# franciscotln/cosmology-model-fit

Hardware: AMD Instinct MI355X
Metric: walker-logL evals/s, Pantheon+ 1701-SN full-cov chi2, theta resident in HBM (higher is better)
Workload: dtype f64; 1 GPU; Pantheon+-shaped 1701-SN full-cov flat-LCDM chi2 + prior, 4096 walkers per GPU per step (BASELINE configs[1] at N=1), G=4000, theta resident in HBM; workload_key=pantheon, walkers_per_gpu=4096, walkers_total=4096, n_sn=1701, n_grid=4000, ndim=4, parallelism=walkers sharded over 1 GPU(s)

## Files before the change

cosmology-model-fit_amd/csrc/cosmofit_api.hip:

```cpp
#include <hip/hip_runtime.h>
#include <sys/prctl.h>

#include <cmath>
#include <cstdio>
#include <cstdlib>
#include <chrono>
#include <cstring>
#include <algorithm>
#include <atomic>
#include <utility>
#include <condition_variable>
#include <memory>
#include <mutex>
#include <string>
#include <thread>
#include <vector>

#include "../../include/cosmofit.h"
#include "cf_pack.h"
#include "cosmofit_device.h"

typedef double d2 __attribute__((ext_vector_type(2)));

#define CF_YPK_SLACK 8192
#define CF_DELTA_SLACK 4096

static long long cf_tune(const char* key, long long dflt) {
  static const std::string env = [] { const char* e = getenv("CF_TUNE"); return std::string(e ? e : ""); }();
  const size_t kl = strlen(key);
  for (size_t pos = 0; pos < env.size();) {
    const size_t end = std::min(env.find(',', pos), env.size());
    if (end - pos > kl + 1 && env.compare(pos, kl, key) == 0 && env[pos + kl] == '=') return atoll(env.c_str() + pos + kl + 1);
    pos = end + 1;
  }
  return dflt;
}

#define CF_BAO_NODES 6
#define CF_SN_PARTS_MAX 4
#define CF_SN_REC_SLACK (512 * CF_SN_PARTS_MAX)
template <int MODEL, int FDE>
__global__ void walker_kernel(cf_dev_desc d, const double* theta, int64_t W, double* delta, double* dm_out, double* mucorr_out,
                              d2* bao_nodes, d2* table_out);
template <int MODEL, int FDE>
__global__ void walker_fast_kernel(cf_walker_args d, const double* theta, int64_t W, double* delta, d2* bao_nodes, double* theta_copy,
                                   int frag_b, int sn_parts);
template <int MODEL, int FDE, int LANES, int ROLES>
__global__ void small_blocks_kernel(cf_dev_desc d, const double* theta, int64_t W, const d2* bao_nodes, double* chi2_extra,
                                    double* blocks_out, double* bao_out);
template <int MODEL, int FDE, int C>
__global__ void growth_kernel(cf_dev_desc d, const double* theta, int64_t W, const d2* aux_nodes, double* chi2_extra, int accumulate,
                              double* blocks_out, double* theory_out);
template <int MODEL, int FDE>
__global__ void hz_kernel(cf_dev_desc d, const double* theta, const double* z, int64_t n, double* out);
#define CF_DECLARE_GROWTH(M, F, C) \
  extern template __global__ void growth_kernel<M, F, C>(cf_dev_desc, const double*, int64_t, const d2*, double*, int, double*, double*);
#define CF_DECLARE_WALKER(M, F)                                                                                            \
  extern template __global__ void walker_kernel<M, F>(cf_dev_desc, const double*, int64_t, double*, double*, double*, d2*, d2*); \
  extern template __global__ void walker_fast_kernel<M, F>(cf_walker_args, const double*, int64_t, double*, d2*, double*, int, int); \
  extern template __global__ void small_blocks_kernel<M, F, 16, 1>(cf_dev_desc, const double*, int64_t, const d2*, double*, \
                                                                   double*, double*);                                      \
  extern template __global__ void small_blocks_kernel<M, F, 64, 1>(cf_dev_desc, const double*, int64_t, const d2*, double*, \
                                                                   double*, double*);                                      \
  extern template __global__ void small_blocks_kernel<M, F, 64, 2>(cf_dev_desc, const double*, int64_t, const d2*, double*, \
                                                                   double*, double*);                                      \
  extern template __global__ void hz_kernel<M, F>(cf_dev_desc, const double*, const double*, int64_t, double*);             \
  CF_DECLARE_GROWTH(M, F, 1) CF_DECLARE_GROWTH(M, F, 2) CF_DECLARE_GROWTH(M, F, 4) CF_DECLARE_GROWTH(M, F, 8)
CF_DECLARE_WALKER(0, 0) CF_DECLARE_WALKER(0, 1) CF_DECLARE_WALKER(0, 2) CF_DECLARE_WALKER(0, 3)
CF_DECLARE_WALKER(1, 0) CF_DECLARE_WALKER(1, 1) CF_DECLARE_WALKER(1, 2) CF_DECLARE_WALKER(1, 3)

typedef void (*walker_fn)(cf_dev_desc, const double*, int64_t, double*, double*, double*, d2*, d2*);
static walker_fn pick_walker(int model, int fde) {
  static const walker_fn table[2][4] = {
      {walker_kernel<0, 0>, walker_kernel<0, 1>, walker_kernel<0, 2>, walker_kernel<0, 3>},
      {walker_kernel<1, 0>, walker_kernel<1, 1>, walker_kernel<1, 2>, walker_kernel<1, 3>}};
  return table[model][fde];
}
typedef void (*walker_fast_fn)(cf_walker_args, const double*, int64_t, double*, d2*, double*, int, int);
static walker_fast_fn pick_walker_fast(int model, int fde) {
  static const walker_fast_fn table[2][4] = {
      {walker_fast_kernel<0, 0>, walker_fast_kernel<0, 1>, walker_fast_kernel<0, 2>, walker_fast_kernel<0, 3>},
      {walker_fast_kernel<1, 0>, walker_fast_kernel<1, 1>, walker_fast_kernel<1, 2>, walker_fast_kernel<1, 3>}};
  return table[model][fde];
}
static bool walker_fast_ok(const cf_dev_desc& d) {
  static const bool off = cf_tune("walker_generic", 0) != 0;
  return !off && d.chunk_shift == 3 && d.ndim <= 64 && !d.sn_fixed_mu && !d.sn_dir && !d.sn_vel_mult && (!d.sn_lin || d.lin_in_rec);
}
static cf_epilogue epilogue_of(const cf_dev_desc& d) {
  cf_epilogue e{};
  e.ndim = d.ndim; e.has_bounds = d.has_bounds; e.n_gauss = d.n_gauss; e.n_chi2_gauss = d.n_chi2_gauss;
  e.cpl_wall = d.cpl_wall; e.n_fs8 = d.n_fs8; e.n_cc = d.n_cc; e.cc_f_inverse = d.cc_f_inverse;
  e.log_norm = d.log_norm; e.logl_const = d.logl_const; e.cc_logdet = d.cc_logdet;
  e.w0 = d.slot[CF_P_W0_D]; e.wa = d.slot[CF_P_WA_D]; e.fs8err = d.slot[CF_P_FS8ERR_D]; e.fcc = d.slot[CF_P_FCC_D];
  for (int k = 0; k < CF_MAX_NDIM; ++k) { e.lo[k] = d.lo[k]; e.hi[k] = d.hi[k]; }
  for (int k = 0; k < CF_MAX_GAUSS; ++k) {
    e.gauss_idx[k] = d.gauss_idx[k]; e.gauss_mean[k] = d.gauss_mean[k]; e.gauss_sigma[k] = d.gauss_sigma[k];
    e.chi2_gauss_idx[k] = d.chi2_gauss_idx[k]; e.chi2_gauss_mean[k] = d.chi2_gauss_mean[k]; e.chi2_gauss_sigma[k] = d.chi2_gauss_sigma[k];
  }
  return e;
}
static cf_walker_args walker_args_of(const cf_dev_desc& d) {
  cf_walker_args a{};
  a.ndim = d.ndim; a.n_grid = d.n_grid; a.ez_model = d.ez_model; a.fde = d.fde;
  a.chunk_shift = d.chunk_shift; a.om_mode = d.om_mode;
  a.n_sn = d.n_sn; a.n_ld = d.n_ld;
  a.has_vstep = d.has_vstep; a.step_pm1 = d.step_pm1; a.lin_in_rec = d.lin_in_rec; a.n_aux = d.n_aux;
  a.z_max = d.z_max; a.step = d.step; a.c = d.c; a.inv_step = d.inv_step; a.inv_last = d.inv_last;
  a.or_h2 = d.or_h2; a.omnu_h2 = d.omnu_h2;
  for (int k = 0; k < CF_N_SLOTS; ++k) a.slot[k] = d.slot[k];
  a.sn_rec = d.sn_rec; a.log10_tab = d.log10_tab; a.nu_sw = d.nu_sw; a.ln_sw = d.ln_sw; a.exp2_tab = d.exp2_tab;
// ... 629 lines not shown
      if (c->solve_mode != CF_SOLVE_BLOCKED_TRSM) {
        cf_pack_inverse(c->sn_chol, c->n_sn, c->sn_chol_ld, prep.ip);
        const double inv_probe = cf_invpack_probe(prep.ip, c->sn_chol, c->sn_chol_ld);
        if (inv_probe <= limit) {
          prep.solve_mode = CF_SOLVE_INVERSE_GEMM;
          prep.probe_rel = inv_probe;
        } else if (c->solve_mode == CF_SOLVE_INVERSE_GEMM) {
          return bail(fail(CF_ERR_ILL_CONDITIONED, "cf_create: the explicit inverse of the factor disagrees with row-by-row forward "
                                                       "substitution by " + fmt_g(inv_probe) + " relative (limit " +
                                                       fmt_g(limit) + "); use CF_SOLVE_BLOCKED_TRSM or CF_SOLVE_AUTO for "
                                                       "this covariance"));
        } else {
          prep.solve_mode = CF_SOLVE_BLOCKED_TRSM;
          prep.ip = cf_host_invpack();
        }
      }
      if (prep.solve_mode == CF_SOLVE_BLOCKED_TRSM) {
        if (pack_default(c->sn_chol, c->n_sn, c->sn_chol_ld, prep.hp, &prep.probe_rel) != 0)
          return bail(fail(CF_ERR_NOT_POSDEF, "cf_create: the Cholesky factor has a non-positive or non-finite pivot"));
        if (!(prep.probe_rel <= CF_PROBE_LIMIT))
          return bail(fail(CF_ERR_ILL_CONDITIONED, "cf_create: the blocked solve disagrees with row-by-row forward substitution by " +
                                                       fmt_g(prep.probe_rel) + " relative on a probe vector (limit 1e-11): "
                                                       "the factor's diagonal blocks are too ill-conditioned for 256-row block inverses"));
      }
      prep.packed = true;
    }
    h->solve_mode = prep.solve_mode;
    h->pack_probe_rel = prep.probe_rel;
    if (h->solve_mode == CF_SOLVE_INVERSE_GEMM) {
      if ((rc = h->ipack.upload(prep.ip))) return bail(rc);
    } else {
      if ((rc = h->pack.upload(prep.hp))) return bail(rc);
    }
  }
  if (c->n_bao > 0) {
    int rc;
    if ((rc = upload_vec(h->bao_z, c->bao_z, c->n_bao))) return bail(rc);
    if ((rc = upload_vec(h->bao_val, c->bao_val, c->n_bao))) return bail(rc);
    if ((rc = upload_vec(h->bao_inv_cov, c->bao_inv_cov, (int64_t)c->n_bao * c->n_bao))) return bail(rc);
    if (h->bao_qty.ensure((size_t)c->n_bao * 4)) return bail(CF_ERR_HIP);
    if (hipMemcpy(h->bao_qty.p, c->bao_qty, (size_t)c->n_bao * 4, hipMemcpyHostToDevice) != hipSuccess)
      return bail(fail(CF_ERR_HIP, "hipMemcpy(bao_qty) failed"));
    d.bao_z = h->bao_z.as<const double>();
    d.bao_val = h->bao_val.as<const double>();
    d.bao_inv_cov = h->bao_inv_cov.as<const double>();
    d.bao_qty = h->bao_qty.as<const int32_t>();
  }
  if (d.n_aux > 0) {
    std::vector<int32_t> base((size_t)d.n_aux);
    for (int k = 0; k < d.n_aux; ++k) base[k] = aux_node_base(d, k < c->n_bao ? c->bao_z[k] : c->fs8_z[k - c->n_bao]);
    if (h->bao_base.ensure(base.size() * 4)) return bail(CF_ERR_HIP);
    if (hipMemcpy(h->bao_base.p, base.data(), base.size() * 4, hipMemcpyHostToDevice) != hipSuccess)
      return bail(fail(CF_ERR_HIP, "hipMemcpy(bao_base) failed"));
    d.bao_base = h->bao_base.as<const int32_t>();
  }
  if (c->n_fs8 > 0) {
    int rc;
    const int n = c->n_fs8;
    if ((rc = upload_vec(h->fs8_z, c->fs8_z, n))) return bail(rc);
    if ((rc = upload_vec(h->fs8_val, c->fs8_val, n))) return bail(rc);
    if ((rc = upload_vec(h->fs8_inv_cov, c->fs8_inv_cov, (int64_t)n * n))) return bail(rc);
    if ((rc = upload_vec(h->fs8_fid, c->fs8_fid, n))) return bail(rc);
    d.fs8_z = h->fs8_z.as<const double>();
    d.fs8_val = h->fs8_val.as<const double>();
    d.fs8_inv_cov = h->fs8_inv_cov.as<const double>();
    d.fs8_fid = h->fs8_fid.as<const double>();
// ... 389 lines not shown
    return a.frag_b ? launch_tri_gemm_small_t<16, true, 1>(a, st) : launch_tri_gemm_small_t<16, false, 1>(a, st);
  }
  if (a.frag_b) return fail(CF_ERR_INVALID, "internal: fragment-ordered residuals handed to the throughput solve kernel");
  return tri_gemm_panel_width(a.W) == 32 ? launch_tri_gemm_t<2, 2>(a, st) : launch_tri_gemm_t<1, 2>(a, st);
}

static int launch_eval(cf_handle* h, const double* th, int64_t Wc, double* out, int out_kind, hipStream_t st,
                       double* dm_out, double* mucorr_out, double* blocks_out, double* bao_out, double* chi2_sn_out,
                       hipEvent_t* ev, double* fs8_block_out = nullptr, double* fs8_theory_out = nullptr) {
  const cf_dev_desc& d = h->d;
  unsigned long long* nf = h->nonfinite.as<unsigned long long>();
  double* delta = h->delta.as<double>();
  d2* bao_nodes = h->bao_nodes.as<d2>();
  if (ev) HIP_TRY(hipEventRecord(ev[0], st));
  if (ev && !(h->d.n_sn > 0 || h->has_small_blocks || h->has_growth || h->qsr)) HIP_TRY(hipEventRecord(ev[1], st));
  const bool walker_work = d.n_sn > 0 || h->has_small_blocks || h->has_growth;
  double* extra = (h->has_small_blocks || h->has_growth || h->qsr) ? h->chi2_extra.as<double>() : nullptr;
  static const bool frag_env = cf_tune("small_frag", 1) != 0;
  const bool small_solve = d.n_sn > 0 && h->solve_mode == CF_SOLVE_INVERSE_GEMM && h->partial4.p && Wc <= small_batch_max();
  const bool frag_b = frag_env && small_solve && !dm_out && !mucorr_out && walker_fast_ok(d) && !h->qsr;
  if (h->qsr) {
    double* th_copy = h->theta_on_host ? h->theta.as<double>() : nullptr;
    int rc = cf_qsr_launch(h->qsr, th, Wc, delta, extra, out_kind, th_copy, st);
    if (rc) return rc;
    if (th_copy) th = th_copy;
    if (ev) HIP_TRY(hipEventRecord(ev[1], st));
  } else if (walker_work) {
    const size_t lds = ((size_t)d.n_grid + (d.n_grid >> d.chunk_shift) + 2) * 16;
    if (!dm_out && !mucorr_out && walker_fast_ok(d)) {
      double* th_copy = h->theta_on_host ? h->theta.as<double>() : nullptr;
      static const int parts_env = (int)cf_tune("sn_parts", 0);
      int sn_parts = parts_env > 0 ? parts_env : (Wc <= 64 ? 4 : (Wc <= 160 ? 2 : 1));
      if (sn_parts > CF_SN_PARTS_MAX || d.n_sn == 0) sn_parts = 1;
      hipLaunchKernelGGL(pick_walker_fast(d.ez_model, d.fde), dim3((unsigned)(Wc * sn_parts)), dim3(512), lds, st, walker_args_of(d), th,
                         Wc, delta, bao_nodes, th_copy, frag_b ? 1 : 0, sn_parts);
      if (th_copy) th = th_copy;
    } else
      hipLaunchKernelGGL(pick_walker(d.ez_model, d.fde), dim3((unsigned)Wc), dim3(512), lds, st, d, th, Wc, delta, dm_out, mucorr_out,
                         bao_nodes, (d2*)nullptr);
    if (ev) HIP_TRY(hipEventRecord(ev[1], st));
    if (h->has_small_blocks) {
      static const int64_t wide_max = cf_tune("sb_wide_max", 2048);
      static const int64_t roles_max = cf_tune("sb_roles_max", 2048);
      const int lanes = Wc <= wide_max ? 64 : 16, roles = (lanes == 64 && Wc <= roles_max) ? 2 : 1, per_wg = 256 / (lanes * roles);
      hipLaunchKernelGGL(pick_small_blocks(d.ez_model, d.fde, lanes, roles), dim3((unsigned)((Wc + per_wg - 1) / per_wg)), dim3(256), 0, st, d, th, Wc,
                         (const d2*)bao_nodes, extra, blocks_out, bao_out);
    }
    if (h->has_growth)
      hipLaunchKernelGGL(pick_growth(d.ez_model, d.fde, d.fs8_steps), dim3((unsigned)Wc), dim3(256),
                         (size_t)(2 * (d.fs8_steps + 1) + 16 + CF_MAX_FS8 + 2 + 256) * 8, st, d, th, Wc, (const d2*)bao_nodes, extra,
                         h->has_small_blocks ? 1 : 0, fs8_block_out, fs8_theory_out);
  }
  if (ev) HIP_TRY(hipEventRecord(ev[2], st));
  if (d.n_sn > 0 && h->solve_mode == CF_SOLVE_INVERSE_GEMM) {
    static const bool trim = cf_tune("gemm_trim", 1) != 0;
    const int n_rb_ = h->ipack.dev.n_rowblocks, nt_last = trim ? std::max(1, std::min(4, (d.n_pad - 64 * (n_rb_ - 1)) / 16)) : 4;
    static const int diag_skip = cf_tune("gemm_diag_skip", 1) != 0;
    TriGemmArgs a{h->epi.as<const cf_epilogue>(), h->ipack.dev.frags, d.n_ld, d.ndim, n_rb_, nt_last, diag_skip, th, Wc, delta,
                  h->max_walkers, h->partial.as<double>(), h->arrivals.as<unsigned int>(), extra, out,
                  out_kind, nf, chi2_sn_out, h->partial4.as<double>(), nullptr, 0ull, frag_b};
    if (h->theta_on_host && h->done_flags.p) {
      a.done_flag = (unsigned long long*)h->done_flags.p;
      a.done_seq = h->done_seq;
      const bool small = Wc <= small_batch_max() && a.partial4;
      const int pw = small ? 16 : tri_gemm_panel_width(Wc);
      h->done_armed = (int)((Wc + pw - 1) / pw);
      if (h->done_armed > CF_DONE_FLAGS) { a.done_flag = nullptr; h->done_armed = 0; }
    }
// ... 820 lines not shown
```

cosmology-model-fit_amd/csrc/cosmofit_device.h:

```cpp
#ifndef COSMOFIT_DEVICE_H
#define COSMOFIT_DEVICE_H

#include <stdint.h>

#define CF_MAX_NDIM 16
#define CF_MAX_GAUSS 8
#define CF_MAX_BAO 64
#define CF_MAX_GL 256
#define CF_MAX_CC 64
#define CF_MAX_FS8 64
#define CF_N_SLOTS 15

#define CF_BLOCK_TILES 16
#define CF_BLOCK_ROWS 256

#define CF_FDE_LCDM_D 0
#define CF_FDE_WCDM_D 1
#define CF_FDE_THAWING_D 2
#define CF_FDE_CPL_D 3

#define CF_EZ_LATE_FLAT_D 0
#define CF_EZ_PHYSICAL_D 1

#define CF_P_OFFSET_D 0
// ... 63 lines not shown
  const double* fs8_pts;
  const double* fs8_tab;
  int32_t n_aux, fs8_n_agrid;
  double or_h2, omnu_h2, o_gamma_h2, nu_m0, nu_rho0;
  double nu_qs_sq[5], nu_ws[5];
  const double* nu_grid;
  const double* ln_grid;
  const double* nu_sw;
  const double* ln_sw;
  const double* exp2_tab;
  int32_t n_bao, bao_dh_exact, rd_from_fit, rd_wm_late;
  const double* bao_z;
  const double* bao_val;
  const double* bao_inv_cov;
  const int32_t* bao_qty;
  const int32_t* bao_base;
  double rd_fit[11];
  int32_t cmb_mode, n_gl;
  const double* gl_x;
  const double* gl_w;
  double cmb_prior[3], cmb_inv_cov[9], zstar_fit[11];
  int32_t has_bounds, n_gauss, n_chi2_gauss, cpl_wall;
  double log_norm;
  int32_t sn_vel_mult, cc_f_inverse;
  double logl_const;
  double lo[CF_MAX_NDIM], hi[CF_MAX_NDIM];
  int32_t gauss_idx[CF_MAX_GAUSS];
  double gauss_mean[CF_MAX_GAUSS], gauss_sigma[CF_MAX_GAUSS];
  int32_t chi2_gauss_idx[CF_MAX_GAUSS];
  double chi2_gauss_mean[CF_MAX_GAUSS], chi2_gauss_sigma[CF_MAX_GAUSS];
};

struct cf_walker_args {
  int32_t ndim, n_grid, ez_model, fde;
  int32_t chunk_shift, om_mode;
  int32_t n_sn, n_ld;
  int32_t has_vstep, step_pm1, lin_in_rec, n_aux;
  double z_max, step, c, inv_step, inv_last;
  double or_h2, omnu_h2;
  cf_dev_slot slot[CF_N_SLOTS];
  const cf_d4* sn_rec;
  const void* log10_tab;
  const double* nu_sw;
  const double* ln_sw;
  const double* exp2_tab;
  const int32_t* bao_base;
};

struct cf_epilogue {
  int32_t ndim, has_bounds, n_gauss, n_chi2_gauss;
  int32_t cpl_wall, n_fs8, n_cc, cc_f_inverse;
  double log_norm, logl_const, cc_logdet;
  cf_dev_slot w0, wa, fs8err, fcc;
  double lo[CF_MAX_NDIM], hi[CF_MAX_NDIM];
  int32_t gauss_idx[CF_MAX_GAUSS];
  double gauss_mean[CF_MAX_GAUSS], gauss_sigma[CF_MAX_GAUSS];
  int32_t chi2_gauss_idx[CF_MAX_GAUSS];
  double chi2_gauss_mean[CF_MAX_GAUSS], chi2_gauss_sigma[CF_MAX_GAUSS];
};
#define CF_EPI_WORDS ((int)((sizeof(cf_epilogue) + 7) / 8))

struct cf_qsr_args {
  int32_t ndim, n_grid;
  int32_t n_sn, n_ld;
  int32_t n_qsr, two_grids;
  int32_t n_bao, n_bz;
  double c, fde_a;
  cf_dev_slot om, w0, h0, off_sn, off_q, scat, rd;
  const double* node_w;
  const double* node_zp3;
  const double* node_lnf;
  const int32_t* sn_j;
  const double* sn_t;
  const double* sn_h;
  const double* sn_zp1;
  const double* sn_obs;
  const int32_t* q_j;
  const double* q_t;
  const double* q_h;
// ... 63 lines not shown
```

cosmology-model-fit_amd/csrc/cosmofit_kernels.hip:

```cpp
#include <hip/hip_runtime.h>
#include <type_traits>
#include <stdint.h>

#include "cosmofit_device.h"
#include "cf_wave_scan.h"

typedef double d4 __attribute__((ext_vector_type(4)));
typedef double d2 __attribute__((ext_vector_type(2)));

#define CF_WAVE 64

__device__ __forceinline__ double slot_get(const cf_dev_desc& d, int s, const double* __restrict__ th) {
  const cf_dev_slot& p = d.slot[s];
  return p.idx >= 0 ? p.scale * th[p.idx] : p.fixed;
}

struct ThetaRow {
  double v;
};
__device__ __forceinline__ double readlane_f64(double v, int lane) {
  return __hiloint2double(__builtin_amdgcn_readlane(__double2hiint(v), lane), __builtin_amdgcn_readlane(__double2loint(v), lane));
}
template <class D>
__device__ __forceinline__ double slot_get(const D& d, int s, const ThetaRow& th) {
// ... 330 lines not shown
    double dx_max = 0.0;
#pragma unroll
    for (int k = 1; k < CH; ++k) {
      const double dx = x[k] - x[k - 1];
      dx_max = fmax(dx_max, fabs(dx));
      double p = fma(dx, 1.0 / 5040, 1.0 / 720);
      p = fma(p, dx, 1.0 / 120);
      p = fma(p, dx, 1.0 / 24);
      p = fma(p, dx, 1.0 / 6);
      p = fma(p, dx, 0.5);
      p = fma(p * dx, dx, dx);
      fde[k] = fma(fde[k - 1], p, fde[k - 1]);
    }
    if (!(dx_max < 0x1p-5)) {
#pragma unroll
      for (int k = 1; k < CH; ++k) fde[k] = exp_tab(x[k], etab);
    }
  }
#pragma unroll
  for (int k = 0; k < CH; ++k) {
    const int g = g0 + k;
    double z = (double)g * d.step;
    if (LAST) z = g >= G - 1 ? d.z_max : z;
    const double e2 = POWER_LAW ? e2_from_fde<MODEL>(wc, z, fde[k], nu_pre[k]) : e2_of_z<MODEL, FDE, true, D>(d, wc, z, nu_pre[k], ln[k], etab);
    const double v = c_over_H0 * rsqrt_pos(e2);
    dh[k] = (LAST && g >= G) ? 0.0 : v;
  }
  double prev = dpp_move<0x138, 0xF>(dh[CH - 1]);
  double run = 0.0;
  const double half = 0.5 * d.step;
#pragma unroll
  for (int k = 0; k < CH; ++k) {
    const bool counts = (k > 0 || lane > 0) && (!LAST || g0 + k < G);
    run = counts ? fma_vsv(prev + dh[k], half, run) : run;
    loc[k] = run;
    prev = dh[k];
  }
  return run;
}

template <int MODEL, int FDE, int CH, class D>
__device__ __forceinline__ void build_distance_table_regs(const D& d, const WalkerCosmo& wc, d2* tab,
                                                          d4* wave_pub, const double (&nu_pre)[CH], const double (&ln_pre)[CH],
                                                          const double* __restrict__ etab) {
  const int G = d.n_grid;
  const int tid = threadIdx.x, lane = tid & 63, wave = tid >> 6;
  const int g0 = tid * CH;
  const int base = g0 + tid;
  const double c_over_H0 = wc.c / wc.H0;
  double dh[CH], loc[CH];
  const int wave_last = (tid - lane) * CH + 64 * CH - 1;
  const double run = wave_last < G - 1 ? chunk_eval<MODEL, FDE, CH, false>(d, wc, c_over_H0, g0, lane, nu_pre, ln_pre, etab, dh, loc)
                                       : chunk_eval<MODEL, FDE, CH, true>(d, wc, c_over_H0, g0, lane, nu_pre, ln_pre, etab, dh, loc);
  const double incl = wave_inclusive_scan(run);
  const double first_dh = __hiloint2double(__builtin_amdgcn_readfirstlane(__double2hiint(dh[0])),
                                           __builtin_amdgcn_readfirstlane(__double2loint(dh[0])));
  if (lane == 63) wave_pub[wave] = (d4){incl, first_dh, dh[CH - 1], 0.0};
  __syncthreads();
  double term = 0.0;
  if (lane < CF_TPB_A / 64) {
    const d4 pv = wave_pub[lane];
    term = lane < wave ? pv[0] : 0.0;
    if (lane >= 1) {
      const int gb = lane * 64 * CH;
      const double zb = gb == G - 1 ? d.z_max : (double)gb * d.step;
      const double bnd = (wave_pub[lane - 1][2] + pv[1]) / 2 * (zb - (double)(gb - 1) * d.step);
      term += (lane <= wave && gb < G) ? bnd : 0.0;
// ... 87 lines not shown
template <class TAB>
__device__ double pchip_dh_tab(const TAB& T, double xi) {
  const int G = T.G;
  if (xi <= 0.0) return T.at(0).y;
  if (xi >= T.z_max) return T.at(G - 1).y;
  int i = (int)(xi * T.inv_step);
  i = i > G - 2 ? G - 2 : i;
  if (i > 0 && grid_z(i, G, T.step, T.z_max) >= xi) --i;
  if (i < G - 2 && grid_z(i + 1, G, T.step, T.z_max) < xi) ++i;
  const double x0 = grid_z(i, G, T.step, T.z_max);
  const double h_i = grid_z(i + 1, G, T.step, T.z_max) - x0;
  const double t = (xi - x0) / h_i;
  const double t2 = t * t, t3 = t2 * t;
  const double h00 = 2 * t3 - 3 * t2 + 1, h10 = t3 - 2 * t2 + t, h01 = -2 * t3 + 3 * t2, h11 = t3 - t2;
  return h00 * T.at(i).y + h10 * h_i * pchip_slope_tab(T, i) + h01 * T.at(i + 1).y + h11 * h_i * pchip_slope_tab(T, i + 1);
}

__device__ double z_star_fit(const double* f, double wb, double wm) {
  wb = pow(wb, f[2]);
  wm = pow(wm, f[3]);
  return pow(wm, f[4]) + f[0] * f[5] * pow(wb, f[6]) * pow(wm, f[7]) + f[1] * f[8] * pow(wm, f[9]) * pow(wb, f[10]);
}
__device__ double r_drag_fit(const double* f, double wb, double wm) {
  wb = pow(wb, f[0]);
  wm = pow(wm, f[1]);
  const double den = (f[2] * pow(wb, f[3])) + (f[4] * pow(wb, f[5]) * pow(wm, f[6])) + (f[7] * pow(wm, f[8]));
  return 1.0 / den - f[9] / pow(wm, f[10]);
}

template <bool FRAG>
__device__ __forceinline__ int delta_index(int i) {
  return FRAG ? ((i >> 3) * 128 + ((i >> 1) & 3) * 32 + (i & 1)) : i;
}
template <bool PM1, bool LIN = false, bool FRAG = false, class D = cf_dev_desc>
__device__ __forceinline__ void sn_fast_loop(const D& d, const DistTable& T, const d2* __restrict__ log_tab,
                                             double* __restrict__ out, double off, double v100, int tid, double lin = 0.0,
                                             int part = 0, int n_parts = 1) {
  const int n_sn = d.n_sn, first = part * CF_TPB_A + tid, stride = n_parts * CF_TPB_A;
  double r_pos = 1.0, r_neg = 1.0, c0 = 0.0;
  if (PM1 && d.has_vstep) {
    r_pos = 1.0 / (1.0 + v100 / d.c);
    r_neg = 1.0 / (1.0 + (-v100) / d.c);
    c0 = -1.0;
  }
  const d4* __restrict__ rec = reinterpret_cast<const d4*>(d.sn_rec) + first;
  if (part == 0 && tid < d.n_ld - n_sn) out[delta_index<FRAG>(n_sn + tid)] = 0.0;
  auto one_sn = [&](const d4& r, int i) {
    const double za = r[0], st = r[1], zhp1 = r[2], ob = r[3];
    double z_cosmo = za;
    if (!LIN && PM1) {
      z_cosmo = fma(za, st > 0.0 ? r_pos : r_neg, c0);
    } else if (!LIN && d.has_vstep) {
      const double z_pec = (v100 * st) / d.c;
      z_cosmo = -1.0 + za / (1.0 + z_pec);
    }
    const double off_i = LIN ? off + lin * st : off;
    out[delta_index<FRAG>(i)] = ob - off_i - fma_vsv(log10_tab(zhp1 * hermite_fast(T, z_cosmo), log_tab), 5.0, 25.0);
  };
  d4 ra = rec[0], rb;
  int i = first;
  while (i < n_sn) {
    rb = rec[stride];
    one_sn(ra, i);
    i += stride;
    if (i >= n_sn) break;
    rec += 2 * stride;
    ra = rec[0];
    one_sn(rb, i);
    i += stride;
  }
}

template <int MODEL, int FDE>
__global__ void __launch_bounds__(CF_TPB_A, 4)
walker_kernel(cf_dev_desc d, const double* __restrict__ theta, int64_t W, double* __restrict__ delta,
              double* __restrict__ dm_out, double* __restrict__ mucorr_out, d2* __restrict__ bao_nodes, d2* __restrict__ table_out) {
  extern __shared__ __align__(16) d2 lds_tab[];
  __shared__ __align__(16) d4 wave_pub[CF_TPB_A / 64];
  __shared__ __align__(16) d2 log_tab[64];
  __shared__ double exp2_tab[64];

  const int64_t w = blockIdx.x;
  if (w >= W) return;
  const double* th = theta + w * d.ndim;
  const int tid = threadIdx.x;
  if (tid < 64 && d.n_sn > 0) log_tab[tid] = reinterpret_cast<const d2*>(d.log10_tab)[tid];
  double nu_pre[8], ln_pre[8];
  constexpr bool POWER_LAW = FDE == CF_FDE_WCDM_D || FDE == CF_FDE_CPL_D;
#pragma unroll
  for (int k = 0; k < 8; ++k) {
    nu_pre[k] = (MODEL == CF_EZ_PHYSICAL_D && d.chunk_shift == 3) ? d.nu_sw[k * CF_TPB_A + tid] : -1.0;
    ln_pre[k] = (POWER_LAW && d.chunk_shift == 3) ? d.ln_sw[k * CF_TPB_A + tid] : -1.0;
  }
  if (POWER_LAW && d.chunk_shift == 3 && tid >= 64 && tid < 128) exp2_tab[tid - 64] = d.exp2_tab[tid - 64];
  if (POWER_LAW && d.chunk_shift == 3) __syncthreads();
  const WalkerCosmo wc = make_cosmo(d, th);
  DistTable T;
  T.tab = lds_tab;
  T.G = d.n_grid;
  T.chs = d.chunk_shift;
  T.step = d.step;
  T.inv_step = d.inv_step;
// ... 27 lines not shown
          double z_cosmo = zc;
          if (d.has_vstep) {
            const double v_km_s = d.sn_dir ? 100 * (d.sn_dir[3 * i] * vx + d.sn_dir[3 * i + 1] * vy + d.sn_dir[3 * i + 2] * vz) * d.sn_step[i]
                                           : v100 * d.sn_step[i];
            const double z_pec = v_km_s / d.c;
            z_cosmo = -1.0 + (1.0 + zc) / (1.0 + z_pec);
            if (d.sn_vel_mult) z_cosmo = fmax((1.0 + zc) * (1.0 + z_pec) - 1.0, 1e-8);
          }
          const double DMc = hermite_tab(T, z_cosmo);
          const double fixed = d.sn_fixed_mu ? d.sn_fixed_mu[i] : __longlong_as_double(0x7ff8000000000000ll);
          if (fixed == fixed) {
            const double DM = hermite_tab(T, zc);
            const double mu_corr = d.has_vstep ? 5.0 * log10_pos(DMc / DM) : 0.0;
            res = d.obs[i] - off_i - mu_corr - fixed;
            if (dm_out) dm_out[w * d.n_sn + i] = DM;
            if (mucorr_out) mucorr_out[w * d.n_sn + i] = mu_corr;
          } else if (!parts) {
            res = d.obs[i] - off_i - (25.0 + 5 * log10_pos((1.0 + d.z_hel[i]) * DMc));
          } else {
            const double DM = hermite_tab(T, zc);
            const double mu_corr = d.has_vstep ? 5.0 * log10(DMc / DM) : 0.0;
            const double mu_th = 25.0 + 5 * log10((1.0 + d.z_hel[i]) * DM);
            res = d.obs[i] - off_i - mu_corr - mu_th;
            if (dm_out) dm_out[w * d.n_sn + i] = DM;
            if (mucorr_out) mucorr_out[w * d.n_sn + i] = mu_corr;
          }
        }
        out[i] = res;
      }
    }
  }
}

template <int MODEL, int FDE>
__global__ void __launch_bounds__(CF_TPB_A, 4)
walker_fast_kernel(cf_walker_args d, const double* __restrict__ theta, int64_t W, double* __restrict__ delta,
                   d2* __restrict__ bao_nodes, double* __restrict__ theta_copy, int frag_b, int sn_parts) {
  extern __shared__ __align__(16) d2 lds_tab[];
  __shared__ __align__(16) d4 wave_pub[CF_TPB_A / 64];
  __shared__ __align__(16) d2 log_tab[64];
  __shared__ double exp2_all[CF_TPB_A / 64][64];

  const int64_t w = sn_parts > 1 ? blockIdx.x / (unsigned)sn_parts : blockIdx.x;
  const int part = sn_parts > 1 ? (int)(blockIdx.x % (unsigned)sn_parts) : 0;
  if (w >= W) return;
  const int tid = threadIdx.x, lane = tid & 63;
  double* const exp2_tab = exp2_all[tid >> 6];
  const ThetaRow th{theta[w * d.ndim + (lane < d.ndim ? lane : 0)]};
  if (theta_copy && part == 0 && tid < d.ndim) theta_copy[w * d.ndim + tid] = th.v;
  constexpr bool POWER_LAW = FDE == CF_FDE_WCDM_D || FDE == CF_FDE_CPL_D;
  d2 lt = (d2){0.0, 0.0};
  double et = 0.0;
  if (tid < 64 && d.n_sn > 0) lt = reinterpret_cast<const d2*>(d.log10_tab)[tid];
  if (POWER_LAW) et = d.exp2_tab[lane];
  double nu_pre[8], ln_pre[8];
#pragma unroll
  for (int k = 0; k < 8; ++k) {
    nu_pre[k] = MODEL == CF_EZ_PHYSICAL_D ? d.nu_sw[k * CF_TPB_A + tid] : -1.0;
    ln_pre[k] = POWER_LAW ? d.ln_sw[k * CF_TPB_A + tid] : -1.0;
  }
  if (tid < 64 && d.n_sn > 0) log_tab[tid] = lt;
  if (POWER_LAW) exp2_tab[lane] = et;
  const WalkerCosmo wc = make_cosmo(d, th);
  const double off = slot_get(d, CF_P_OFFSET_D, th);
  const double v100 = 100 * slot_get(d, CF_P_V_D, th);
  const double lin = d.lin_in_rec ? slot_get(d, CF_P_LIN_D, th) : 0.0;
  DistTable T;
  T.tab = lds_tab;
  T.G = d.n_grid;
  T.chs = 3;
  T.step = d.step;
  T.inv_step = d.inv_step;
  T.inv_last = d.inv_last;
  T.z_max = d.z_max;
  build_distance_table_regs<MODEL, FDE, 8>(d, wc, lds_tab, wave_pub, nu_pre, ln_pre, exp2_tab);
  for (int e = CF_TPB_A - 1 - tid; part == 0 && e < CF_BAO_NODES * d.n_aux; e += CF_TPB_A) {
    const int k = e / CF_BAO_NODES, o = e % CF_BAO_NODES;
    bao_nodes[(w * d.n_aux + k) * CF_BAO_NODES + o] = T.at(d.bao_base[k] + o);
  }
  if (d.n_sn > 0 && !frag_b) {
    double* out = delta + w * d.n_ld;
    if (d.lin_in_rec) sn_fast_loop<false, true>(d, T, log_tab, out, off, v100, tid, lin, part, sn_parts);
    else if (d.step_pm1) sn_fast_loop<true>(d, T, log_tab, out, off, v100, tid, 0.0, part, sn_parts);
    else sn_fast_loop<false>(d, T, log_tab, out, off, v100, tid, 0.0, part, sn_parts);
  } else if (d.n_sn > 0) {
    double* out = delta + (w >> 4) * (16 * (int64_t)d.n_ld) + 2 * (w & 15);
    if (d.lin_in_rec) sn_fast_loop<false, true, true>(d, T, log_tab, out, off, v100, tid, lin, part, sn_parts);
    else if (d.step_pm1) sn_fast_loop<true, false, true>(d, T, log_tab, out, off, v100, tid, 0.0, part, sn_parts);
    else sn_fast_loop<false, false, true>(d, T, log_tab, out, off, v100, tid, 0.0, part, sn_parts);
  }
}

template <int MODEL, int FDE>
__device__ __forceinline__ double H_at_gl_node(const cf_dev_desc& d, const WalkerCosmo& wc, double z, const double* __restrict__ etab,
                                               const d2* __restrict__ ltab) {
  const double zp1 = 1.0 + z;
  const double cubed = zp1 * zp1 * zp1;
  double f = 1.0;
  if (FDE == CF_FDE_WCDM_D) {
    f = exp_tab((3 * (1 + wc.w0)) * (log10_tab(zp1, ltab) * 2.30258509299404568402), etab);
  } else if (FDE == CF_FDE_CPL_D) {
    f = exp_tab(fma(3 * (1 + wc.w0 + wc.wa), log10_tab(zp1, ltab) * 2.30258509299404568402, div_pos(-3 * wc.wa * z, zp1)), etab);
  } else if (FDE == CF_FDE_THAWING_D) {
    const double r = div_pos(2 * cubed, (1.0 + wc.w0) + (1.0 - wc.w0) * cubed);
    f = r * r;
  }
  double e2;
  if (MODEL == CF_EZ_LATE_FLAT_D) {
    e2 = (FDE == CF_FDE_LCDM_D) ? wc.Om * cubed + (1.0 - wc.Om) : wc.Om * cubed + (1.0 - wc.Om) * f;
  } else {
    const double de = (FDE == CF_FDE_LCDM_D) ? wc.Ode : wc.Ode * f;
    const double r = div_pos(d.nu_m0, zp1), mz_sq = r * r;
    const double ws = sqrt_pos(d.nu_qs_sq[0] + mz_sq) * d.nu_ws[0] + sqrt_pos(d.nu_qs_sq[1] + mz_sq) * d.nu_ws[1] +
                      sqrt_pos(d.nu_qs_sq[2] + mz_sq) * d.nu_ws[2] + sqrt_pos(d.nu_qs_sq[3] + mz_sq) * d.nu_ws[3] +
                      sqrt_pos(d.nu_qs_sq[4] + mz_sq) * d.nu_ws[4];
    const double zp1_2 = zp1 * zp1;
    const double nu = div_pos(zp1_2 * zp1_2 * ws, d.nu_rho0);
    e2 = wc.Or * (cubed * zp1) + wc.Obc * cubed + de + wc.Onu * nu;
  }
  return wc.H0 * sqrt_pos(e2);
}

template <int LANES>
__device__ __forceinline__ double group_sum(double v) {
// ... 469 lines not shown
  __syncthreads();
  double tj = 0.0;
  if (lane < n) {
    const double* col = d.fs8_inv_cov + lane;
#pragma unroll 4
    for (int i = wave; i < n; i += 4) tj += resid[i] * col[i * n];
  }
  part[wave * 64 + lane] = tj;
  __syncthreads();
  if (wave != 0) return;
  double r_own = lane < n ? (((part[lane] + part[64 + lane]) + part[128 + lane]) + part[192 + lane]) * resid[lane] : 0.0;
#pragma unroll
  for (int off = 32; off > 0; off >>= 1) r_own += __shfl_xor(r_own, off);
  if (lane == 0) {
    const double c = r_own * (ferr * ferr);
    chi2_extra[w] = accumulate ? chi2_extra[w] + c : c;
    if (blocks_out) blocks_out[w] = c;
  }
}

template <int MODEL, int FDE>
__global__ void hz_kernel(cf_dev_desc d, const double* __restrict__ theta, const double* __restrict__ z, int64_t n,
                          double* __restrict__ out) {
  const int64_t i = blockIdx.x * (int64_t)blockDim.x + threadIdx.x;
  if (i >= n) return;
  const WalkerCosmo wc = make_cosmo(d, theta);
  out[i] = H_of_z<MODEL, FDE>(d, wc, z[i]);
}

#define CF_INSTANTIATE_GROWTH(M, F, C) \
  template __global__ void growth_kernel<M, F, C>(cf_dev_desc, const double*, int64_t, const d2*, double*, int, double*, double*);
#define CF_INSTANTIATE_WALKER(M, F)                                                                              \
  template __global__ void walker_kernel<M, F>(cf_dev_desc, const double*, int64_t, double*, double*, double*, d2*, d2*); \
  template __global__ void walker_fast_kernel<M, F>(cf_walker_args, const double*, int64_t, double*, d2*, double*, int, int);     \
  template __global__ void small_blocks_kernel<M, F, 16, 1>(cf_dev_desc, const double*, int64_t, const d2*, double*, double*, \
                                                            double*);                                                      \
  template __global__ void small_blocks_kernel<M, F, 64, 1>(cf_dev_desc, const double*, int64_t, const d2*, double*, double*, \
                                                            double*);                                                      \
  template __global__ void small_blocks_kernel<M, F, 64, 2>(cf_dev_desc, const double*, int64_t, const d2*, double*, double*, \
                                                            double*);                                                      \
  template __global__ void hz_kernel<M, F>(cf_dev_desc, const double*, const double*, int64_t, double*);                     \
  CF_INSTANTIATE_GROWTH(M, F, 1) CF_INSTANTIATE_GROWTH(M, F, 2) CF_INSTANTIATE_GROWTH(M, F, 4) CF_INSTANTIATE_GROWTH(M, F, 8)
CF_INSTANTIATE_WALKER(0, 0) CF_INSTANTIATE_WALKER(0, 1) CF_INSTANTIATE_WALKER(0, 2) CF_INSTANTIATE_WALKER(0, 3)
CF_INSTANTIATE_WALKER(1, 0) CF_INSTANTIATE_WALKER(1, 1) CF_INSTANTIATE_WALKER(1, 2) CF_INSTANTIATE_WALKER(1, 3)

__device__ __forceinline__ double epi_slot(const cf_dev_slot& sl, const double* __restrict__ th) {
  return sl.idx >= 0 ? th[sl.idx] * sl.scale : sl.fixed;
}
__device__ __forceinline__ double finalize_value(const cf_epilogue& d, const double* __restrict__ th, double chi2, int out_kind,
                                                 unsigned long long* nonfinite) {
  for (int g = 0; g < d.n_chi2_gauss; ++g) {
    double diff = th[d.chi2_gauss_idx[g]] - d.chi2_gauss_mean[g];
    chi2 += diff * diff / (d.chi2_gauss_sigma[g] * d.chi2_gauss_sigma[g]);
  }
  if (out_kind == CF_OUT_CHI2_D) return chi2;
  double lp = 0.0;
  if (out_kind == CF_OUT_LOGP_D) {
    if (d.has_bounds) {
      bool inbox = true;
      for (int k0 = 0; k0 < d.ndim; k0 += 4) {
#pragma unroll
        for (int k = k0; k < k0 + 4; ++k) {
          const double t = th[k < d.ndim ? k : 0];
          inbox = inbox & ((k >= d.ndim) | ((d.lo[k & (CF_MAX_NDIM - 1)] < t) & (t < d.hi[k & (CF_MAX_NDIM - 1)])));
        }
      }
      if (!inbox) return -INFINITY;
// ... 804 lines not shown
```

Baseline: 18.19 million evals/s.

## Preload SN records early in walker_fast kernel and pin kernel args in SGPRs

```diff
diff --git a/cosmology-model-fit_amd/csrc/cosmofit_api.hip b/cosmology-model-fit_amd/csrc/cosmofit_api.hip
--- a/cosmology-model-fit_amd/csrc/cosmofit_api.hip
+++ b/cosmology-model-fit_amd/csrc/cosmofit_api.hip
@@ -43,8 +43,8 @@
 __global__ void walker_kernel(cf_dev_desc d, const double* theta, int64_t W, double* delta, double* dm_out, double* mucorr_out,
                               d2* bao_nodes, d2* table_out);
 template <int MODEL, int FDE>
-__global__ void walker_fast_kernel(cf_walker_args d, const double* theta, int64_t W, double* delta, d2* bao_nodes, double* theta_copy,
-                                   int frag_b, int sn_parts);
+__global__ void walker_fast_kernel(double* delta, d2* bao_nodes, cf_walker_args d, const double* theta, int64_t W, double* theta_copy,
+                                   int sn_parts, int frag_b);
 template <int MODEL, int FDE, int LANES, int ROLES>
 __global__ void small_blocks_kernel(cf_dev_desc d, const double* theta, int64_t W, const d2* bao_nodes, double* chi2_extra,
                                     double* blocks_out, double* bao_out);
@@ -57,7 +57,7 @@
   extern template __global__ void growth_kernel<M, F, C>(cf_dev_desc, const double*, int64_t, const d2*, double*, int, double*, double*);
 #define CF_DECLARE_WALKER(M, F)                                                                                            \
   extern template __global__ void walker_kernel<M, F>(cf_dev_desc, const double*, int64_t, double*, double*, double*, d2*, d2*); \
-  extern template __global__ void walker_fast_kernel<M, F>(cf_walker_args, const double*, int64_t, double*, d2*, double*, int, int); \
+  extern template __global__ void walker_fast_kernel<M, F>(double*, d2*, cf_walker_args, const double*, int64_t, double*, int, int); \
   extern template __global__ void small_blocks_kernel<M, F, 16, 1>(cf_dev_desc, const double*, int64_t, const d2*, double*, \
                                                                    double*, double*);                                      \
   extern template __global__ void small_blocks_kernel<M, F, 64, 1>(cf_dev_desc, const double*, int64_t, const d2*, double*, \
@@ -76,7 +76,7 @@
       {walker_kernel<1, 0>, walker_kernel<1, 1>, walker_kernel<1, 2>, walker_kernel<1, 3>}};
   return table[model][fde];
 }
-typedef void (*walker_fast_fn)(cf_walker_args, const double*, int64_t, double*, d2*, double*, int, int);
+typedef void (*walker_fast_fn)(double*, d2*, cf_walker_args, const double*, int64_t, double*, int, int);
 static walker_fast_fn pick_walker_fast(int model, int fde) {
   static const walker_fast_fn table[2][4] = {
       {walker_fast_kernel<0, 0>, walker_fast_kernel<0, 1>, walker_fast_kernel<0, 2>, walker_fast_kernel<0, 3>},
@@ -772,6 +772,15 @@
     } else {
       if ((rc = h->pack.upload(prep.hp))) return bail(rc);
     }
+  } else {
+    const std::vector<cf_d4> rec((size_t)CF_SN_REC_SLACK, cf_d4{1.0, 1.0, 1.0, 0.0});
+    if (h->sn_rec.ensure(rec.size() * sizeof(cf_d4))) return bail(CF_ERR_HIP);
+    if (hipMemcpy(h->sn_rec.p, rec.data(), rec.size() * sizeof(cf_d4), hipMemcpyHostToDevice) != hipSuccess)
+      return bail(fail(CF_ERR_HIP, "hipMemcpy(sn_rec) failed"));
+    d.sn_rec = h->sn_rec.as<const cf_d4>();
+    int rc;
+    if ((rc = upload_log10_table(h->log10_tab))) return bail(rc);
+    d.log10_tab = h->log10_tab.p;
   }
   if (c->n_bao > 0) {
     int rc;
@@ -1227,8 +1236,8 @@
       static const int parts_env = (int)cf_tune("sn_parts", 0);
       int sn_parts = parts_env > 0 ? parts_env : (Wc <= 64 ? 4 : (Wc <= 160 ? 2 : 1));
       if (sn_parts > CF_SN_PARTS_MAX || d.n_sn == 0) sn_parts = 1;
-      hipLaunchKernelGGL(pick_walker_fast(d.ez_model, d.fde), dim3((unsigned)(Wc * sn_parts)), dim3(512), lds, st, walker_args_of(d), th,
-                         Wc, delta, bao_nodes, th_copy, frag_b ? 1 : 0, sn_parts);
+      hipLaunchKernelGGL(pick_walker_fast(d.ez_model, d.fde), dim3((unsigned)(Wc * sn_parts)), dim3(512), lds, st, delta, bao_nodes,
+                         walker_args_of(d), th, Wc, th_copy, sn_parts, frag_b ? 1 : 0);
       if (th_copy) th = th_copy;
     } else
       hipLaunchKernelGGL(pick_walker(d.ez_model, d.fde), dim3((unsigned)Wc), dim3(512), lds, st, d, th, Wc, delta, dm_out, mucorr_out,
diff --git a/cosmology-model-fit_amd/csrc/cosmofit_device.h b/cosmology-model-fit_amd/csrc/cosmofit_device.h
--- a/cosmology-model-fit_amd/csrc/cosmofit_device.h
+++ b/cosmology-model-fit_amd/csrc/cosmofit_device.h
@@ -119,19 +119,20 @@
 };
 
 struct cf_walker_args {
-  int32_t ndim, n_grid, ez_model, fde;
-  int32_t chunk_shift, om_mode;
-  int32_t n_sn, n_ld;
-  int32_t has_vstep, step_pm1, lin_in_rec, n_aux;
-  double z_max, step, c, inv_step, inv_last;
+  const int32_t* bao_base;
+  double inv_step, inv_last;
+  int32_t n_aux, n_ld;
+  int32_t has_vstep, step_pm1, lin_in_rec, chunk_shift;
+  int32_t fde, ez_model, om_mode, ndim;
+  int32_t n_sn, n_grid;
+  double z_max, step, c;
   double or_h2, omnu_h2;
-  cf_dev_slot slot[CF_N_SLOTS];
   const cf_d4* sn_rec;
   const void* log10_tab;
   const double* nu_sw;
   const double* ln_sw;
   const double* exp2_tab;
-  const int32_t* bao_base;
+  cf_dev_slot slot[CF_N_SLOTS];
 };
 
 struct cf_epilogue {
diff --git a/cosmology-model-fit_amd/csrc/cosmofit_kernels.hip b/cosmology-model-fit_amd/csrc/cosmofit_kernels.hip
--- a/cosmology-model-fit_amd/csrc/cosmofit_kernels.hip
+++ b/cosmology-model-fit_amd/csrc/cosmofit_kernels.hip
@@ -386,7 +386,8 @@
 #pragma unroll
   for (int k = 0; k < CH; ++k) {
     const bool counts = (k > 0 || lane > 0) && (!LAST || g0 + k < G);
-    run = counts ? fma_vsv(prev + dh[k], half, run) : run;
+    const double upd = fma_vsv(prev + dh[k], half, run);
+    run = counts ? upd : run;
     loc[k] = run;
     prev = dh[k];
   }
@@ -540,10 +541,19 @@
 __device__ __forceinline__ int delta_index(int i) {
   return FRAG ? ((i >> 3) * 128 + ((i >> 1) & 3) * 32 + (i & 1)) : i;
 }
-template <bool PM1, bool LIN = false, bool FRAG = false, class D = cf_dev_desc>
+template <int NPRE>
+__device__ __forceinline__ void sn_preload(const cf_d4* sn_rec, int n_sn, int tid, int part, int n_parts, d4 (&pre)[NPRE]) {
+  const int first = part * CF_TPB_A + tid, stride = n_parts * CF_TPB_A;
+  const d4* __restrict__ rec = reinterpret_cast<const d4*>(sn_rec) + first;
+  pre[0] = rec[0];
+#pragma unroll
+  for (int k = 1; k < NPRE; ++k) pre[k] = rec[first + (k - 1) * stride < n_sn ? k * stride : 0];
+}
+
+template <bool PM1, bool LIN = false, bool FRAG = false, int NPRE = 0, class D = cf_dev_desc>
 __device__ __forceinline__ void sn_fast_loop(const D& d, const DistTable& T, const d2* __restrict__ log_tab,
                                              double* __restrict__ out, double off, double v100, int tid, double lin = 0.0,
-                                             int part = 0, int n_parts = 1) {
+                                             int part = 0, int n_parts = 1, d4* pre = nullptr) {
   const int n_sn = d.n_sn, first = part * CF_TPB_A + tid, stride = n_parts * CF_TPB_A;
   double r_pos = 1.0, r_neg = 1.0, c0 = 0.0;
   if (PM1 && d.has_vstep) {
@@ -565,17 +575,31 @@
     const double off_i = LIN ? off + lin * st : off;
     out[delta_index<FRAG>(i)] = ob - off_i - fma_vsv(log10_tab(zhp1 * hermite_fast(T, z_cosmo), log_tab), 5.0, 25.0);
   };
-  d4 ra = rec[0], rb;
   int i = first;
-  while (i < n_sn) {
-    rb = rec[stride];
-    one_sn(ra, i);
-    i += stride;
-    if (i >= n_sn) break;
-    rec += 2 * stride;
-    ra = rec[0];
-    one_sn(rb, i);
-    i += stride;
+  if constexpr (NPRE > 0) {
+    static_assert(NPRE == 2, "sn_fast_loop: two preloaded records, or none");
+    auto turn = [&](d4& r) {
+      if (i >= n_sn) return false;
+      one_sn(r, i);
+      if (i + NPRE * stride < n_sn) r = rec[NPRE * stride];
+      rec += stride;
+      i += stride;
+      return true;
+    };
+    while (turn(pre[0]) && turn(pre[1])) {
+    }
+  } else {
+    d4 ra = rec[0], rb;
+    while (i < n_sn) {
+      rb = rec[stride];
+      one_sn(ra, i);
+      i += stride;
+      if (i >= n_sn) break;
+      rec += 2 * stride;
+      ra = rec[0];
+      one_sn(rb, i);
+      i += stride;
+    }
   }
 }
 
@@ -669,14 +693,38 @@
   }
 }
 
+#define CF_PIN(...) asm volatile("" ::__VA_ARGS__)
+#define CF_PIN_SLOT(p) CF_PIN("s"((p).idx), "s"((p).scale), "s"((p).fixed))
 template <int MODEL, int FDE>
 __global__ void __launch_bounds__(CF_TPB_A, 4)
-walker_fast_kernel(cf_walker_args d, const double* __restrict__ theta, int64_t W, double* __restrict__ delta,
-                   d2* __restrict__ bao_nodes, double* __restrict__ theta_copy, int frag_b, int sn_parts) {
+walker_fast_kernel(double* __restrict__ delta, d2* __restrict__ bao_nodes, cf_walker_args d, const double* __restrict__ theta, int64_t W,
+                   double* __restrict__ theta_copy, int sn_parts, int frag_b) {
   extern __shared__ __align__(16) d2 lds_tab[];
   __shared__ __align__(16) d4 wave_pub[CF_TPB_A / 64];
   __shared__ __align__(16) d2 log_tab[64];
   __shared__ double exp2_all[CF_TPB_A / 64][64];
+
+  constexpr bool POWER_LAW = FDE == CF_FDE_WCDM_D || FDE == CF_FDE_CPL_D;
+  constexpr bool PHYSICAL = MODEL == CF_EZ_PHYSICAL_D;
+  constexpr int NPRE = 2;
+  CF_PIN("s"(sn_parts), "s"(W), "s"(theta), "s"(theta_copy), "s"(d.ndim), "s"(d.n_sn), "s"(d.n_grid), "s"(d.ez_model), "s"(d.sn_rec),
+         "s"(d.log10_tab), "s"(d.z_max), "s"(d.step), "s"(d.c),
+         "s"(delta), "s"(bao_nodes), "s"(d.bao_base), "s"(frag_b), "s"(d.n_aux), "s"(d.n_ld), "s"(d.has_vstep), "s"(d.step_pm1),
+         "s"(d.lin_in_rec), "s"(d.inv_step));
+  CF_PIN_SLOT(d.slot[CF_P_OFFSET_D]);
+  CF_PIN_SLOT(d.slot[CF_P_H0_D]);
+  CF_PIN_SLOT(d.slot[CF_P_V_D]);
+  if constexpr (!PHYSICAL) {
+    CF_PIN("s"(d.om_mode));
+    CF_PIN_SLOT(d.slot[CF_P_OM_D]);
+  } else {
+    CF_PIN("s"(d.nu_sw), "s"(d.or_h2), "s"(d.omnu_h2));
+    CF_PIN_SLOT(d.slot[CF_P_OBH2_D]);
+    CF_PIN_SLOT(d.slot[CF_P_OCH2_D]);
+  }
+  if constexpr (FDE != CF_FDE_LCDM_D) CF_PIN_SLOT(d.slot[CF_P_W0_D]);
+  if constexpr (FDE == CF_FDE_CPL_D) CF_PIN_SLOT(d.slot[CF_P_WA_D]);
+  if constexpr (POWER_LAW) CF_PIN("s"(d.ln_sw), "s"(d.exp2_tab));
 
   const int64_t w = sn_parts > 1 ? blockIdx.x / (unsigned)sn_parts : blockIdx.x;
   const int part = sn_parts > 1 ? (int)(blockIdx.x % (unsigned)sn_parts) : 0;
@@ -684,24 +732,26 @@
   const int tid = threadIdx.x, lane = tid & 63;
   double* const exp2_tab = exp2_all[tid >> 6];
   const ThetaRow th{theta[w * d.ndim + (lane < d.ndim ? lane : 0)]};
-  if (theta_copy && part == 0 && tid < d.ndim) theta_copy[w * d.ndim + tid] = th.v;
-  constexpr bool POWER_LAW = FDE == CF_FDE_WCDM_D || FDE == CF_FDE_CPL_D;
   d2 lt = (d2){0.0, 0.0};
   double et = 0.0;
-  if (tid < 64 && d.n_sn > 0) lt = reinterpret_cast<const d2*>(d.log10_tab)[tid];
+  if (tid < 64) lt = reinterpret_cast<const d2*>(d.log10_tab)[tid];
   if (POWER_LAW) et = d.exp2_tab[lane];
   double nu_pre[8], ln_pre[8];
 #pragma unroll
   for (int k = 0; k < 8; ++k) {
-    nu_pre[k] = MODEL == CF_EZ_PHYSICAL_D ? d.nu_sw[k * CF_TPB_A + tid] : -1.0;
+    nu_pre[k] = PHYSICAL ? d.nu_sw[k * CF_TPB_A + tid] : -1.0;
     ln_pre[k] = POWER_LAW ? d.ln_sw[k * CF_TPB_A + tid] : -1.0;
   }
-  if (tid < 64 && d.n_sn > 0) log_tab[tid] = lt;
+  d4 pre[NPRE];
+  __builtin_amdgcn_sched_barrier(0);
+  sn_preload<NPRE>(d.sn_rec, d.n_sn, tid, part, sn_parts, pre);
   if (POWER_LAW) exp2_tab[lane] = et;
   const WalkerCosmo wc = make_cosmo(d, th);
   const double off = slot_get(d, CF_P_OFFSET_D, th);
   const double v100 = 100 * slot_get(d, CF_P_V_D, th);
   const double lin = d.lin_in_rec ? slot_get(d, CF_P_LIN_D, th) : 0.0;
+  if (theta_copy && part == 0 && tid < d.ndim) theta_copy[w * d.ndim + tid] = th.v;
+  if (tid < 64) log_tab[tid] = lt;
   DistTable T;
   T.tab = lds_tab;
   T.G = d.n_grid;
@@ -717,16 +767,18 @@
   }
   if (d.n_sn > 0 && !frag_b) {
     double* out = delta + w * d.n_ld;
-    if (d.lin_in_rec) sn_fast_loop<false, true>(d, T, log_tab, out, off, v100, tid, lin, part, sn_parts);
-    else if (d.step_pm1) sn_fast_loop<true>(d, T, log_tab, out, off, v100, tid, 0.0, part, sn_parts);
-    else sn_fast_loop<false>(d, T, log_tab, out, off, v100, tid, 0.0, part, sn_parts);
+    if (d.lin_in_rec) sn_fast_loop<false, true, false, NPRE>(d, T, log_tab, out, off, v100, tid, lin, part, sn_parts, pre);
+    else if (d.step_pm1) sn_fast_loop<true, false, false, NPRE>(d, T, log_tab, out, off, v100, tid, 0.0, part, sn_parts, pre);
+    else sn_fast_loop<false, false, false, NPRE>(d, T, log_tab, out, off, v100, tid, 0.0, part, sn_parts, pre);
   } else if (d.n_sn > 0) {
     double* out = delta + (w >> 4) * (16 * (int64_t)d.n_ld) + 2 * (w & 15);
-    if (d.lin_in_rec) sn_fast_loop<false, true, true>(d, T, log_tab, out, off, v100, tid, lin, part, sn_parts);
-    else if (d.step_pm1) sn_fast_loop<true, false, true>(d, T, log_tab, out, off, v100, tid, 0.0, part, sn_parts);
-    else sn_fast_loop<false, false, true>(d, T, log_tab, out, off, v100, tid, 0.0, part, sn_parts);
-  }
-}
+    if (d.lin_in_rec) sn_fast_loop<false, true, true, NPRE>(d, T, log_tab, out, off, v100, tid, lin, part, sn_parts, pre);
+    else if (d.step_pm1) sn_fast_loop<true, false, true, NPRE>(d, T, log_tab, out, off, v100, tid, 0.0, part, sn_parts, pre);
+    else sn_fast_loop<false, false, true, NPRE>(d, T, log_tab, out, off, v100, tid, 0.0, part, sn_parts, pre);
+  }
+}
+#undef CF_PIN_SLOT
+#undef CF_PIN
 
 template <int MODEL, int FDE>
 __device__ __forceinline__ double H_at_gl_node(const cf_dev_desc& d, const WalkerCosmo& wc, double z, const double* __restrict__ etab,
@@ -1262,7 +1314,7 @@
   template __global__ void growth_kernel<M, F, C>(cf_dev_desc, const double*, int64_t, const d2*, double*, int, double*, double*);
 #define CF_INSTANTIATE_WALKER(M, F)                                                                              \
   template __global__ void walker_kernel<M, F>(cf_dev_desc, const double*, int64_t, double*, double*, double*, d2*, d2*); \
-  template __global__ void walker_fast_kernel<M, F>(cf_walker_args, const double*, int64_t, double*, d2*, double*, int, int);     \
+  template __global__ void walker_fast_kernel<M, F>(double*, d2*, cf_walker_args, const double*, int64_t, double*, int, int);     \
   template __global__ void small_blocks_kernel<M, F, 16, 1>(cf_dev_desc, const double*, int64_t, const d2*, double*, double*, \
                                                             double*);                                                      \
   template __global__ void small_blocks_kernel<M, F, 64, 1>(cf_dev_desc, const double*, int64_t, const d2*, double*, double*, \
```

Result: no change. 18.15 million evals/s (-0.2%).
